# SudYar/MLVectorDB

Hardware: AMD Instinct MI355X
Metric: queries/sec, exact cosine kNN k=10 over a row-sharded Nx768 fp32 corpus (10M rows per GPU) (higher is better)
Workload: dtype i8 (MFMA bounds) + f64 (exact rescoring of the f32 rows)

## Files before the change

### mlvectordb_amd/csrc/kernels_filter.hip

```cpp
#include <cstdlib>
#include <type_traits>

#include "bound_common.h"
#include "internal.h"
#include "query_norm.h"
#include "scan_common.h"

namespace mlvdb {

typedef __bf16 bf16x8 __attribute__((ext_vector_type(8)));
typedef float f32x4 __attribute__((ext_vector_type(4)));
typedef int i32x4 __attribute__((ext_vector_type(4)));
typedef float f32x8 __attribute__((ext_vector_type(8)));
typedef unsigned int u32x4 __attribute__((ext_vector_type(4)));

__device__ __forceinline__ __amdgpu_buffer_rsrc_t make_rsrc(const void* base, uint32_t bytes) {
    return __builtin_amdgcn_make_buffer_rsrc(const_cast<void*>(base), 0, bytes, 0x00020000);
}
__device__ __forceinline__ float4 buf_load_f4(__amdgpu_buffer_rsrc_t r, uint32_t voff, uint32_t soff) {
    return __builtin_bit_cast(float4, __builtin_amdgcn_raw_buffer_load_b128(r, voff, soff, 0));
}
__device__ __forceinline__ float4 buf_load_f4_nt(__amdgpu_buffer_rsrc_t r, uint32_t voff, uint32_t soff) {
    return __builtin_bit_cast(float4, __builtin_amdgcn_raw_buffer_load_b128(r, voff, soff, 2));
}
// ... 1564 lines not shown
        const float v = x * invf;
        const __bf16 b = (__bf16)v;
        int kc = c >> 6, ks, g, j;
        if (a.Xb) {
            ks = (c >> 5) & 1; g = (c >> 3) & 3; j = c & 7;
        } else {
            const int t = (c >> 4) & 3;
            ks = t >> 1; g = (c >> 2) & 3; j = (t & 1) * 4 + (c & 3);
        }
        if (want_bf16) img[((((int64_t)kc * 16 + n16) * 2 + ks) * 64 + (c16 + 16 * g)) * 8 + j] = b;
        if (c < dim) {
            const double e = (double)x * inv - (double)(float)(__bf16)(x * invf);
            e2 = __builtin_fma(e, e, e2);
        }
        amax = __builtin_fmaxf(amax, __builtin_fabsf(v));
    }
    for (int off = 32; off > 0; off >>= 1) {
        e2 += __shfl_xor(e2, off);
        amax = __builtin_fmaxf(amax, __shfl_xor(amax, off));
    }
    __syncthreads();
    if (lane == 0) {
        dred[wave] = e2;
        fred[wave] = amax;
    }
    __syncthreads();
    if (threadIdx.x == 0) {
        float e = (float)(__builtin_sqrt((dred[0] + dred[1]) + (dred[2] + dred[3])) * 1.000001);
        e = float_bump(e);
        if (real) qerr[q] = e;
        const double nrm = live ? (a.space == kSpaceCosine ? 0.0 : qaux[q]) : 0.0;
        a.qscale[q] = a.space == kSpaceL2 ? (float)(2.0 * nrm) : 1.0f;
        const double e1q = (real ? (double)e : 0.0) + 1.00390625 * (double)*a.row_err + (double)ld * 2.384185791015625e-07;
        const float ke = (float)(e1q * 1.000001) + (a.space == kSpaceCosine ? 2.0f : 1.0f) * kSlack;
        a.ke[q] = float_bump(ke);
        a.thr[q] = real ? -3.0e38f : 3.4e38f;
        a.cnt[q] = 0;
        a.overflow[q] = s_flag ? 1u : 0u;
    }
    if (!want_i8) return;
    amax = __builtin_fmaxf(__builtin_fmaxf(fred[0], fred[1]), __builtin_fmaxf(fred[2], fred[3]));
    if (a.l2c) {
        if (threadIdx.x == 0) a.rmaxq[q] = live ? float_above((double)amax * (qaux[q] + 1e-30) * 1.000001) : 0.f;
        return;
    }
    const float sq = amax > 0.f ? amax / 127.0f : 1.0f;
    const float isq = 1.0f / sq;
    int8_t* img8 = reinterpret_cast<int8_t*>(a.qimg8);
    double err2 = 0.0;
    for (int c = threadIdx.x; c < a.ld8; c += 256) {
        const float v = live && c < ld ? dst[c] * invf : 0.f;
        float t = __builtin_rintf(v * isq);
        t = __builtin_fminf(127.f, __builtin_fmaxf(-127.f, t));
        const double e = (double)v - (double)sq * (double)t;
        err2 += e * e;
        const int kc = c >> 7, ks = (c >> 6) & 1, g = (c >> 4) & 3, j = c & 15;
        img8[((((int64_t)kc * 16 + n16) * 2 + ks) * 64 + (c16 + 16 * g)) * 16 + j] = (int8_t)t;
    }
    for (int off = 32; off > 0; off >>= 1) err2 += __shfl_xor(err2, off);
    __syncthreads();
    if (lane == 0) dred[wave] = err2;
    __syncthreads();
    if (threadIdx.x == 0) {
        const double eq8 = __builtin_sqrt(dred[0] + dred[1] + dred[2] + dred[3]) * 1.000001 + 1e-12;
        a.sq8[q] = sq;
        a.ke8[q] = real ? float_above(eq8) : 0.f;
        if (real && a.nq > 1) {
            atomicMin(a.sqmin, __float_as_uint(sq));
            atomicMax(a.sqmin + 1, __float_as_uint(float_above(eq8)));
        }
        if (real && a.nq == 1) {
            prep8_fin_query(a, 0, sq, float_above(eq8));
        }
    }
    if (want_i8 && a.nq == 1 && q > 0 && threadIdx.x == 0) prep8_fin_query(a, q, 1.0f, 0.0f);
}

__global__ __launch_bounds__(256) void filter_prep8_l2c_kernel(const FilterArgs a) {
    __shared__ double dred[4];
    const int q = blockIdx.x;
    const int ld = a.ld;
    const int lane = threadIdx.x & 63, wave = threadIdx.x >> 6;
    const bool real = q < a.nq;
    __shared__ __attribute__((aligned(16))) unsigned long long s_key[kFilterQueries];
    __shared__ float s_q[2];
    const float rmax_t = (int)threadIdx.x < a.nq ? a.rmaxq[threadIdx.x] : -1.f;
    {
        const unsigned long long key = rank_key_256(rmax_t, (int)threadIdx.x);
        s_key[threadIdx.x] = key;
        __syncthreads();
        if (rmax_t >= 0.f && rank_among_256(s_key, key) == (a.nq - 1) / 2) s_q[0] = rmax_t;
    }
    __syncthreads();
    {
        const float cap = s_q[0] > 0.f ? 4.0f * s_q[0] : 3.0e38f;
        float v = rmax_t;
        v = (v >= 0.f && v <= cap) ? v : 0.f;
        for (int off = 32; off > 0; off >>= 1) v = __builtin_fmaxf(v, __shfl_xor(v, off));
        if ((threadIdx.x & 63) == 0) dred[threadIdx.x >> 6] = (double)v;
    }
    __syncthreads();
    float qmax = (float)__builtin_fmax(__builtin_fmax(dred[0], dred[1]), __builtin_fmax(dred[2], dred[3]));
    __syncthreads();
    if (qmax > 0.f && qmax < 1.0e30f) {
        float g = exp2f(ceilf(log2f(qmax) * 4.0f) * 0.25f);
        if (g < qmax) g *= 1.18920712f;
        if (g >= qmax && g <= qmax * 1.5f) qmax = g;
    }
    const float SQ = qmax > 0.f ? float_above((double)qmax * (2.0 / 127.0) * 1.000001) : 1.0f;
    const bool live = real && a.overflow[q] == 0u;
    const double nrm = live ? a.qaux[q] : 0.0;
    const float invf = (float)(1.0 / (nrm + 1e-30));
    const float sq = nrm > 0.0 ? (float)((double)SQ / (2.0 * nrm)) : 1.0f;
    const float isq = 1.0f / sq;
    int8_t* img8 = reinterpret_cast<int8_t*>(a.qimg8);
    const int n16 = q >> 4, c16 = q & 15;
    double err2 = 0.0;
    for (int c = threadIdx.x; c < a.ld8; c += 256) {
        const float v = live && c < ld ? a.Qpad[(int64_t)q * ld + c] * invf : 0.f;
        float t = __builtin_rintf(v * isq);
        t = __builtin_fminf(127.f, __builtin_fmaxf(-127.f, t));
        const double e = (double)v - (double)sq * (double)t;
        err2 += e * e;
        const int kc = c >> 7, ks = (c >> 6) & 1, g = (c >> 4) & 3, j = c & 15;
        img8[((((int64_t)kc * 16 + n16) * 2 + ks) * 64 + (c16 + 16 * g)) * 16 + j] = (int8_t)t;
    }
    for (int off = 32; off > 0; off >>= 1) err2 += __shfl_xor(err2, off);
    if (lane == 0) dred[wave] = err2;
    __syncthreads();
    if (threadIdx.x == 0) {
        const double eq8 = __builtin_sqrt(dred[0] + dred[1] + dred[2] + dred[3]) * 1.000001 + 1e-12;
        a.sq8[q] = sq;
        a.ke8[q] = real ? float_above(eq8) : 0.f;
        prep8_fin_query(a, q, 1.0f, 0.0f);
    }
}

hipError_t launch_filter_prep_fused(const FilterArgs& a, const float* queries, int32_t dim, float* Qpad, double* qaux, float* qerr,
                                    hipStream_t s) {
    const int want_i8 = a.X8 != nullptr;
    if (!want_i8 && !filter_supported(a.ld)) return hipErrorInvalidValue;
    filter_prep_fused_kernel<<<kFilterQueries, 256, 0, s>>>(a, queries, dim, Qpad, qaux, qerr, want_i8);
    if (want_i8 && a.l2c) filter_prep8_l2c_kernel<<<kFilterQueries, 256, 0, s>>>(a);
    else if (want_i8 && a.nq > 1) filter_prep8_fin_kernel<<<1, kFilterQueries, 0, s>>>(a, 1);
    return hipGetLastError();
}

hipError_t launch_filter_prep8(const FilterArgs& a, hipStream_t s) {
    filter_prep8_kernel<<<kFilterQueries, 256, 0, s>>>(a);
    filter_prep8_fin_kernel<<<1, kFilterQueries, 0, s>>>(a, 1);
    return hipGetLastError();
}

__device__ __forceinline__ uint32_t radix_select_atleast256(const uint32_t* keys, uint32_t cnt, uint32_t want, uint32_t cap,
                                                            uint32_t kmin, uint32_t kmax, uint32_t* hist, uint32_t* s_sel,
                                                            uint32_t* ties, uint32_t* total) {
    const int lane = threadIdx.x & 63, wave = threadIdx.x >> 6;
    const uint32_t want0 = want;
    const uint32_t diff = kmin ^ kmax;
    uint32_t prefix = kmax, mask = 0xffffffffu;
    if (diff != 0) {
        const int hb = 31 - __builtin_clz(diff);
        mask = hb == 31 ? 0u : ~((2u << hb) - 1u);
        prefix = kmax & mask;
        int shift = hb >= 7 ? hb - 7 : 0, width = hb - shift + 1;
        for (;;) {
            __syncthreads();
            hist[threadIdx.x] = 0;
            __syncthreads();
            const uint32_t dmask = (1u << width) - 1u;
            for (uint32_t idx = threadIdx.x; idx < cnt; idx += 256) {
                const uint32_t key = keys[idx];
                if (key != 0 && (key & mask) == prefix) atomicAdd(&hist[(key >> shift) & dmask], 1u);
            }
            __syncthreads();
            if (wave == 0) {
                const uint32_t h0 = hist[4 * lane], h1 = hist[4 * lane + 1], h2 = hist[4 * lane + 2], h3 = hist[4 * lane + 3];
                uint32_t above = h0 + h1 + h2 + h3;
                uint32_t run = above;
                for (int off = 1; off < 64; off <<= 1) {
                    const uint32_t v = __shfl_down(run, off);
                    if (lane + off < 64) run += v;
                }
                above = run - above;
                const uint32_t c3 = above + h3, c2 = c3 + h2, c1 = c2 + h1, c0 = c1 + h0;
                if (above < want && c0 >= want) {
                    if (c3 >= want) { s_sel[0] = 4 * lane + 3; s_sel[1] = above; s_sel[2] = h3; }
                    else if (c2 >= want) { s_sel[0] = 4 * lane + 2; s_sel[1] = c3; s_sel[2] = h2; }
                    else if (c1 >= want) { s_sel[0] = 4 * lane + 1; s_sel[1] = c2; s_sel[2] = h1; }
                    else { s_sel[0] = 4 * lane; s_sel[1] = c1; s_sel[2] = h0; }
                }
            }
            __syncthreads();
            prefix |= s_sel[0] << shift;
            mask |= dmask << shift;
            want -= s_sel[1];
            if (want0 - want + s_sel[2] <= cap) {
                *ties = 0xffffffffu;
                *total = want0 - want + s_sel[2];
                return prefix;
            }
            if (shift == 0) break;
            const int next = shift >= 8 ? shift - 8 : 0;
            width = shift - next;
            shift = next;
        }
        *ties = want;
        *total = want0;
        return prefix;
    }
    *ties = want;
    *total = want0;
    return prefix;
}

template <int kPer>
__global__ __launch_bounds__(256) void filter_prefix_thr_kernel(const FilterArgs a, const double* __restrict__ d64, const int32_t m,
                                                                const int32_t k) {
    __shared__ __attribute__((aligned(16))) uint32_t tmax[256];
    __shared__ uint32_t sel[256];
    __shared__ uint32_t s_n[4];
    const int q = blockIdx.x;
    const double aux = a.qaux[q];
    if (a.l2c && a.overflow[q]) return;
    if (a.space == kSpaceIp && !(aux > 0.0)) return;
    uint32_t key[kPer], best = 0;
    double dk[kPer];
#pragma unroll
    for (int j = 0; j < kPer; ++j) {
        const int i = j * 256 + threadIdx.x;
        dk[j] = i < m ? d64[(int64_t)q * m + i] : __builtin_inf();
    }
#pragma unroll
    for (int j = 0; j < kPer; ++j) {
        key[j] = 0;
        if (dk[j] < 1.0e300) {
            double s;
            if (a.space == kSpaceCosine) s = 1.0 - dk[j];
            else if (a.space == kSpaceIp) s = (1.0 - dk[j]) / aux;
            else s = aux * aux - dk[j];
            const double mag = a.space == kSpaceL2 ? aux * aux + __builtin_fabs(dk[j]) : __builtin_fabs(s) + 1.0;
            key[j] = float_order_key(float_below(s - 1e-9 * mag));
            if (key[j] == 0) key[j] = 1;
            best = max(best, key[j]);
        }
    }
    tmax[threadIdx.x] = best;
    if (threadIdx.x < 4) s_n[threadIdx.x] = 0;
    __syncthreads();
    if (k <= 256) {
        uint32_t rank = 0;
        const uint4* t4 = reinterpret_cast<const uint4*>(tmax);
        const uint32_t me = threadIdx.x;
#pragma unroll 8
        for (uint32_t j = 0; j < 64; ++j) {
            const uint4 o = t4[j];
            rank += (o.x > best || (o.x == best && 4 * j < me)) ? 1u : 0u;
            rank += (o.y > best || (o.y == best && 4 * j + 1 < me)) ? 1u : 0u;
            rank += (o.z > best || (o.z == best && 4 * j + 2 < me)) ? 1u : 0u;
            rank += (o.w > best || (o.w == best && 4 * j + 3 < me)) ? 1u : 0u;
        }
        if (rank == (uint32_t)k - 1u) s_n[1] = best;
    }
    __syncthreads();
    const uint32_t L = s_n[1];
    if (L == 0) return;
#pragma unroll
    for (int j = 0; j < kPer; ++j)
        if (key[j] >= L) {
            const uint32_t pos = atomicAdd(&s_n[0], 1u);
            if (pos < 256u) sel[pos] = key[j];
        }
    __syncthreads();
    const uint32_t n = s_n[0];
    uint32_t tkey = L;
    if (n <= 256u) {
        if (threadIdx.x < n) {
            const uint32_t mine = sel[threadIdx.x];
            uint32_t rank = 0;
            for (uint32_t j = 0; j < n; ++j) {
                const uint32_t o = sel[j];
                rank += (o > mine || (o == mine && j < threadIdx.x)) ? 1u : 0u;
            }
            if (rank == (uint32_t)k - 1u) s_n[2] = mine;
        }
        __syncthreads();
        tkey = s_n[2];
    }
    if (threadIdx.x == 0) a.thr[q] = float_from_order_key(tkey);
}

hipError_t launch_filter_prefix_thr(const FilterArgs& a, const double* d64, int32_t m, int32_t k, hipStream_t s) {
    if (m < 1 || m > 3 * kSeedRows || k < 1 || k > 256) return hipErrorInvalidValue;
    if (m <= kSeedRows) filter_prefix_thr_kernel<kSeedRows / 256><<<a.nq, 256, 0, s>>>(a, d64, m, k);
    else filter_prefix_thr_kernel<3 * kSeedRows / 256><<<a.nq, 256, 0, s>>>(a, d64, m, k);
    return hipGetLastError();
}

struct FinishOut {
    int32_t q0;
    int64_t* labels;
    float* dist;
    int32_t* counts;
    double* d64;
    unsigned long long* rescored;
    int32_t* qsel;
    int32_t* nflag;
};

template <int SPACE, bool FINISH = false>
__global__ __launch_bounds__(256) void filter_refine_thr_kernel(const FilterArgs a, const int32_t k, const int32_t forced_cnt,
                                                                const bool fuse, const int32_t picks, const FinishOut fo) {
    extern __shared__ __attribute__((aligned(16))) char smem[];
    double* qs = reinterpret_cast<double*>(smem);
    double* sc = qs + a.ld;
    double* smin = sc + 64;
    int32_t* pick = reinterpret_cast<int32_t*>(smin + 1);
    uint32_t* hist = reinterpret_cast<uint32_t*>(pick + 64);
    uint32_t* s_scan = hist + 256;
    uint32_t* keys = s_scan + 24;
    CandEntry* stage = reinterpret_cast<CandEntry*>(keys + kCandCap);
    const int q = blockIdx.x;
    if (FINISH && blockIdx.x == 0 && fo.qsel) {
        uint32_t* s_flagged = s_scan + 18;
        const int t = threadIdx.x;
        const bool flagged = t < a.nq && (a.overflow[t] != 0 || a.cnt[t] > (uint32_t)kCandCap);
        const unsigned long long bal = __ballot(flagged);
        if ((t & 63) == 0) s_flagged[t >> 6] = __popcll(bal);
        __syncthreads();
        int base = 0;
        for (int w = 0; w < (t >> 6); ++w) base += (int)s_flagged[w];
        if (flagged) fo.qsel[base + __popcll(bal & ((1ull << (t & 63)) - 1ull))] = t;
        if (t == 0) {
            const int n = (int)(s_flagged[0] + s_flagged[1] + s_flagged[2] + s_flagged[3]);
            *fo.nflag = n;
            if (fo.rescored) fo.rescored[1] += (unsigned long long)n;
        }
    }
    if (q >= a.nq || a.overflow[q]) return;
    const uint32_t cnt = forced_cnt >= 0 ? (uint32_t)forced_cnt : a.cnt[q];
    if (cnt > (uint32_t)kCandCap) {
        if (fuse && threadIdx.x == 0) a.overflow[q] = 1u;
        return;
    }
    bool ok = cnt >= (uint32_t)k && k <= 64;
    if (!ok && !fuse) return;
    const int ld = a.ld;
    const int lane = threadIdx.x & 63, wave = threadIdx.x >> 6;
    CandEntry* list = a.cand + (int64_t)q * kCandCap;
    for (int c = threadIdx.x; c < ld; c += 256) qs[c] = (double)a.Qpad[(int64_t)q * ld + c];
    uint32_t n_valid = 0, kmin = 0xffffffffu, kmax = 0;
    for (uint32_t base = 0; base < cnt; base += 256 * 8) {
        CandEntry e[8];
#pragma unroll
        for (int j = 0; j < 8; ++j) {
            const uint32_t idx = base + j * 256 + threadIdx.x;
            e[j] = list[idx < cnt ? idx : cnt - 1];
        }
#pragma unroll
        for (int j = 0; j < 8; ++j) {
            const uint32_t idx = base + j * 256 + threadIdx.x;
            if (idx >= cnt) continue;
            if (fuse) stage[idx] = e[j];
            uint32_t key = 0;
            if (e[j].u == e[j].u) {
                key = float_order_key(e[j].u);
                if (key == 0) key = 1;
                ++n_valid;
                kmin = min(kmin, key);
                kmax = max(kmax, key);
            }
            keys[idx] = key;
        }
    }
    for (int off = 32; off > 0; off >>= 1) {
        n_valid += __shfl_xor(n_valid, off);
        kmin = min(kmin, (uint32_t)__shfl_xor(kmin, off));
        kmax = max(kmax, (uint32_t)__shfl_xor(kmax, off));
    }
    if (lane == 0) {
        s_scan[wave] = n_valid;
        s_scan[4 + wave] = kmin;
        s_scan[8 + wave] = kmax;
    }
    __syncthreads();
    n_valid = s_scan[0] + s_scan[1] + s_scan[2] + s_scan[3];
    kmin = min(min(s_scan[4], s_scan[5]), min(s_scan[6], s_scan[7]));
    kmax = max(max(s_scan[8], s_scan[9]), max(s_scan[10], s_scan[11]));
    if (n_valid < (uint32_t)k) ok = false;
    uint32_t m = 0;
    if (ok) {
        const uint32_t want = min((uint32_t)max(picks, k), 64u), cap = max(want, 32u);
        uint32_t tkey = 1, ties = 0xffffffffu;
        m = n_valid;
        if (n_valid > cap) tkey = radix_select_atleast256(keys, cnt, want, cap, kmin, kmax, hist, s_scan + 12, &ties, &m);
        if (threadIdx.x == 0) s_scan[16] = 0;
        __syncthreads();
        const bool split = ties != 0xffffffffu;
        for (uint32_t idx = threadIdx.x; idx < cnt; idx += 256) {
            const uint32_t key = keys[idx];
            if (key != 0 && (split ? key > tkey : key >= tkey)) {
                const uint32_t pos = atomicAdd(&s_scan[16], 1u);
                if (pos < 64u) pick[pos] = fuse ? stage[idx].row : list[idx].row;
            }
        }
        if (split && wave == 0) {
            uint32_t taken = 0;
            const uint32_t above = m - ties;
            for (uint32_t base = 0; base < cnt && taken < ties; base += 64) {
                const uint32_t idx = base + lane;
                const bool hit = idx < cnt && keys[idx] == tkey;
                const unsigned long long bal = __ballot(hit);
                const uint32_t pos = taken + (uint32_t)__popcll(bal & ((1ull << lane) - 1ull));
                if (hit && pos < ties && above + pos < 64u) pick[above + pos] = fuse ? stage[idx].row : list[idx].row;
                taken += (uint32_t)__popcll(bal);
            }
        }
    }
    __syncthreads();
    if (ok) m = min(m, 64u);
    const int rslot = threadIdx.x >> 3, l8 = threadIdx.x & 7;
    const double qinv = a.qaux[q];
    const int ngroups = ld >> 4;
    constexpr int G = 6;
    for (uint32_t p0 = 0; p0 < m; p0 += 32) {
        const uint32_t pidx = p0 + rslot;
        const bool have = pidx < m;
        const int32_t row = have ? pick[pidx] : pick[0];
        const float* rb = a.X + (int64_t)(row >> 4) * (kPanelRows * ld) + (row & 15) * 16;
        double acc = 0.0, nx = 0.0;
        for (int c0 = l8; c0 < ngroups; c0 += 8 * G) {
            float4 v[G][4];
#pragma unroll
            for (int j = 0; j < G; ++j) {
                const int cg = c0 + 8 * j < ngroups ? c0 + 8 * j : c0;
                const float4* src = reinterpret_cast<const float4*>(rb + (int64_t)cg * kGroupFloats);
#pragma unroll
                for (int i = 0; i < 4; ++i) v[j][i] = src[i];
            }
#pragma unroll
            for (int j = 0; j < G; ++j) {
                if (c0 + 8 * j >= ngroups) continue;
                const double* qp = qs + (c0 + 8 * j) * 16;
#pragma unroll
                for (int i = 0; i < 4; ++i) {
                    const double x[4] = {(double)v[j][i].x, (double)v[j][i].y, (double)v[j][i].z, (double)v[j][i].w};
#pragma unroll
                    for (int t = 0; t < 4; ++t) {
                        if (SPACE == kSpaceL2) {
                            const double e = qp[4 * i + t] - x[t];
                            acc = __builtin_fma(e, e, acc);
                        } else {
                            acc = __builtin_fma(qp[4 * i + t], x[t], acc);
                        }
                        if (SPACE == kSpaceCosine) nx = __builtin_fma(x[t], x[t], nx);
                    }
                }
            }
        }
        for (int off = 1; off < 8; off <<= 1) {
            acc += __shfl_xor(acc, off);
            if (SPACE == kSpaceCosine) nx += __shfl_xor(nx, off);
        }
        const double dk = finish_distance<SPACE>(acc, nx, qinv);
        double s;
        if (SPACE == kSpaceCosine) s = 1.0 - dk;
        else if (SPACE == kSpaceIp) s = (1.0 - dk) / qinv;
        else s = qinv * qinv - dk;
        if (have && l8 == 0) sc[pidx] = s == s ? s : -__builtin_inf();
    }
    if (threadIdx.x == 0) *smin = -__builtin_inf();
    __syncthreads();
    if (ok && threadIdx.x < m) {
        const double si = sc[threadIdx.x];
        uint32_t rank = 0;
        for (uint32_t j = 0; j < m; ++j) {
            const double sj = sc[j];
            rank += (sj > si || (sj == si && j < threadIdx.x)) ? 1u : 0u;
        }
        if (rank == (uint32_t)k - 1u) *smin = si;
    }
    __syncthreads();
    float thr = a.thr[q];
    if (ok) {
        const double sm = *smin;
        if (sm > -1.0e300 && sm < 1.0e300) {
            const double mag = SPACE == kSpaceL2 ? qinv * qinv + __builtin_fabs(sm) : __builtin_fabs(sm) + 1.0;
            const float t = float_below(sm - 1e-9 * mag);
            if (t > thr) thr = t;
        }
    }
    if (!fuse) {
        if (threadIdx.x == 0) a.thr[q] = thr;
        return;
    }
    const uint32_t per = ((cnt + 255u) / 256u) * 64u;
    const uint32_t wb = min(cnt, (uint32_t)wave * per), we = min(cnt, wb + per);
    uint32_t keep = 0;
    for (uint32_t base = wb; base < we; base += 64) {
        const uint32_t idx = base + lane;
        keep += (uint32_t)__popcll(__ballot(idx < we && stage[idx].u >= thr));
    }
    if (lane == 0) s_scan[wave] = keep;
    __syncthreads();
    uint32_t pos = 0;
    for (int w = 0; w < wave; ++w) pos += s_scan[w];
    const uint32_t new_cnt = s_scan[0] + s_scan[1] + s_scan[2] + s_scan[3];
    uint32_t* surv = keys;
    if (FINISH || new_cnt != cnt) {
        for (uint32_t base = wb; base < we; base += 64) {
            const uint32_t idx = base + lane;
            const bool kept = idx < we && stage[idx].u >= thr;
            const unsigned long long bal = __ballot(kept);
            const uint32_t at = pos + (uint32_t)__popcll(bal & ((1ull << lane) - 1ull));
            if (kept) {
                if (FINISH) surv[at] = (uint32_t)stage[idx].row;
                else list[at] = stage[idx];
            }
            pos += (uint32_t)__popcll(bal);
        }
    }
    if (threadIdx.x == 0) {
        a.thr[q] = thr;
        a.cnt[q] = new_cnt;
    }
    if (!FINISH) return;
    __syncthreads();
    constexpr int kFinWaves = 4;
    double* ed = reinterpret_cast<double*>(stage);
    int32_t* el = reinterpret_cast<int32_t*>(ed + kRescoreRankMax);
    RangeHit* rs = a.rs + (int64_t)q * kCandCap;
    const bool in_lds = new_cnt <= (uint32_t)kRescoreRankMax;
    {
        const int g = lane >> 4, r = lane & 15;
        for (uint32_t base = (uint32_t)wave * 16; base < new_cnt; base += kFinWaves * 16) {
            const uint32_t idx = base + r;
            const bool have = idx < new_cnt;
            const int32_t row = (int32_t)surv[have ? idx : base];
            const float* rbase[1] = {a.X + (int64_t)(row >> 4) * (kPanelRows * ld) + (row & 15) * 16 + g * 4};
            double acc[1][1], nx[1];
            accumulate_rows<SPACE, 1, 1, kRescorePF>(rbase, qs, ld, g, acc, nx);
            const double dist = finish_distance<SPACE>(acc[0][0], nx[0], qinv);
            if (have && lane < 16) {
                const float nrm = a.rn[row];
                const bool live = nrm == nrm;
                if (in_lds) {
                    ed[idx] = live ? dist : __builtin_inf();
                    el[idx] = live ? row : kNoLabel;
                } else {
                    RangeHit hit;
                    hit.d = live ? dist : __builtin_inf();
                    hit.l = live ? row : kNoLabel;
                    hit.pad = 0;
                    rs[idx] = hit;
                }
            }
        }
    }
    if (threadIdx.x == 0) s_scan[17] = 0;
    __syncthreads();
    const int64_t o = (int64_t)(fo.q0 + q) * k;
    if (in_lds) {
        int mine = 0;
        for (uint32_t i = wave; i < new_cnt; i += kFinWaves) {
            const double di = ed[i];
            const int32_t li = el[i];
            if (li == kNoLabel) continue;
            ++mine;
            int rank = 0;
            for (uint32_t j0 = 0; j0 < new_cnt && rank < k; j0 += 128) {
                const uint32_t j = j0 + lane, j2 = j + 64;
                const bool l0 = j < new_cnt && entry_less(ed[j], el[j], di, li);
                const bool l1 = j2 < new_cnt && entry_less(ed[j2], el[j2], di, li);
                rank += __popcll(__ballot(l0)) + __popcll(__ballot(l1));
            }
            if (lane == 0 && rank < k) {
                fo.labels[o + rank] = (int64_t)li;
                fo.dist[o + rank] = (float)di;
                if (fo.d64) fo.d64[o + rank] = di;
            }
        }
        if (lane == 0 && mine) atomicAdd(&s_scan[17], (uint32_t)mine);
        __syncthreads();
        const int n_out = min((int)s_scan[17], k);
        for (int i = n_out + threadIdx.x; i < k; i += 256) {
            fo.labels[o + i] = -1;
            fo.dist[o + i] = __builtin_inff();
            if (fo.d64) fo.d64[o + i] = __builtin_inf();
        }
        if (threadIdx.x == 0) {
            fo.counts[fo.q0 + q] = n_out;
            if (fo.rescored) atomicAdd(fo.rescored, (unsigned long long)new_cnt);
        }
        return;
    }
    double* sd = reinterpret_cast<double*>(stage);
    int32_t* sl = reinterpret_cast<int32_t*>(sd + kFinWaves * 64);
    WaveTopK top;
    top.init();
    for (uint32_t b = 0; b < new_cnt; b += kFinWaves * 64) {
        const uint32_t i = b + wave * 64 + lane;
        RangeHit hh;
        hh.d = __builtin_inf();
        hh.l = kNoLabel;
        if (i < new_cnt) hh = rs[i];
        top.offer(hh.l != kNoLabel, hh.d, hh.l, k, lane);
    }
    sd[wave * 64 + lane] = top.d;
    sl[wave * 64 + lane] = top.l;
    __syncthreads();
    if (wave != 0) return;
    WaveTopK f;
    f.init();
#pragma unroll
    for (int w2 = 0; w2 < kFinWaves; ++w2)
        f.offer(lane < k && sl[w2 * 64 + lane] != kNoLabel, sd[w2 * 64 + lane], sl[w2 * 64 + lane], k, lane);
    const bool valid = lane < k && f.l != kNoLabel;
    if (lane < k) {
        fo.labels[o + lane] = valid ? (int64_t)f.l : -1;
        fo.dist[o + lane] = valid ? (float)f.d : __builtin_inff();
        if (fo.d64) fo.d64[o + lane] = valid ? f.d : __builtin_inf();
    }
    const int n_valid_out = __popcll(__ballot(valid));
    if (lane == 0) {
        fo.counts[fo.q0 + q] = n_valid_out;
        if (fo.rescored) atomicAdd(fo.rescored, (unsigned long long)new_cnt);
    }
}

bool filter_refine_can_fuse(const FilterArgs& a) { return a.ld <= 2048; }

hipError_t launch_filter_refine_thr(const FilterArgs& a, int32_t k, int32_t forced_cnt, bool fuse, hipStream_t s) {
    const size_t lds = (size_t)a.ld * sizeof(double) + 65 * sizeof(double) + 64 * 4 + 256 * 4 + 24 * 4 + (size_t)kCandCap * 4 +
                       (fuse ? (size_t)kCandCap * sizeof(CandEntry) : 0);
    auto kern = a.space == kSpaceL2 ? filter_refine_thr_kernel<kSpaceL2>
                : a.space == kSpaceCosine ? filter_refine_thr_kernel<kSpaceCosine> : filter_refine_thr_kernel<kSpaceIp>;
    static std::atomic<uint64_t> configured[3];
    if (hipError_t e = ensure_dynamic_lds(configured[a.space], reinterpret_cast<const void*>(kern), 160 * 1024); e != hipSuccess)
        return e;
    const int pv = a.tn ? a.tn->refine_picks : 0;
    int picks = pv > 0 ? pv : k + k / 2;
    if (pv <= 0 && picks < 16) picks = 16;
    picks = picks < k ? k : (picks > 64 ? 64 : picks);
    kern<<<a.nq, 256, lds, s>>>(a, k, forced_cnt, fuse, picks, FinishOut{});
    return hipGetLastError();
}

hipError_t launch_filter_finish_small(const FilterArgs& a, int32_t k, int32_t q0, int64_t* out_labels, float* out_dist,
                                      int32_t* out_counts, double* out_d64, unsigned long long* rescored, int32_t* qsel,
                                      int32_t* nflag, hipStream_t s) {
    if (!filter_refine_can_fuse(a) || k < 1 || k > 64) return hipErrorInvalidValue;
    const size_t lds = (size_t)a.ld * sizeof(double) + 65 * sizeof(double) + 64 * 4 + 256 * 4 + 24 * 4 + (size_t)kCandCap * 4 +
                       (size_t)kCandCap * sizeof(CandEntry);
    auto kern = a.space == kSpaceL2 ? filter_refine_thr_kernel<kSpaceL2, true>
                : a.space == kSpaceCosine ? filter_refine_thr_kernel<kSpaceCosine, true> : filter_refine_thr_kernel<kSpaceIp, true>;
    static std::atomic<uint64_t> configured[3];
    if (hipError_t e = ensure_dynamic_lds(configured[a.space], reinterpret_cast<const void*>(kern), 160 * 1024); e != hipSuccess)
        return e;
    const int pv = a.tn ? a.tn->refine_picks : 0;
    int picks = pv > 0 ? pv : k + k / 2;
    if (pv <= 0 && picks < 16) picks = 16;
    picks = picks < k ? k : (picks > 64 ? 64 : picks);
    FinishOut fo{q0, out_labels, out_dist, out_counts, out_d64, rescored, qsel, nflag};
    kern<<<a.nq, 256, lds, s>>>(a, k, -1, true, picks, fo);
    return hipGetLastError();
}

template <int SPACE, bool XB, bool DENSE = false>
static hipError_t launch_scan_one(const FilterArgs& a, int64_t row_begin, int64_t row_end, hipStream_t s) {
    constexpr int NW = 4, MT = 2;
    constexpr int tile_rows = NW * 16 * MT;
    const int64_t tile_begin = row_begin / tile_rows;
    const int64_t tile_end = (row_end + tile_rows - 1) / tile_rows;
    if (tile_end <= tile_begin) return hipSuccess;
    const size_t lds = 2 * kChunkVec * sizeof(uint4) + 3 * kFilterQueries * sizeof(float) +
                       (size_t)NW * 4 * MT * 64 * sizeof(float);
    const int64_t ntiles = tile_end - tile_begin;
    const int max_grid = 256 * 2;
    const int grid = (int)(ntiles < max_grid ? ntiles : max_grid);
    auto kern = filter_scan_kernel<SPACE, XB, DENSE>;
    static std::atomic<uint64_t> configured{0};
    if (hipError_t e = ensure_dynamic_lds(configured, reinterpret_cast<const void*>(kern), (int)lds); e != hipSuccess)
        return e;
    kern<<<grid, NW * 64, lds, s>>>(a, tile_begin, tile_end);
    return hipGetLastError();
}

constexpr int kNarrowMaxQueries = 64;
constexpr size_t kNarrowLdsMax = 152 * 1024;
static int narrow_nqt(int nq) { return nq <= 16 ? 1 : (nq <= 32 ? 2 : 4); }
static size_t narrow_lds(int32_t ld, int nqt, int nw, bool i8 = false) {
    return (size_t)(ld / (i8 ? 64 : 32)) * nqt * 1024 + 3 * kFilterQueries * sizeof(float) + (size_t)nw * 4 * 2 * 64 * sizeof(float);
}
bool filter_narrow_ok(const FilterArgs& a) {
    if (!a.Xb || a.X8 || a.nq > kNarrowMaxQueries) return false;
    if (a.tn->scan_narrow == 0) return false;
    return narrow_lds(a.ld, narrow_nqt(a.nq), 8) <= kNarrowLdsMax;
}
template <int SPACE, int NQT, bool DENSE, int R, int NW, bool I8 = false>
static hipError_t launch_scan_narrow_n(const FilterArgs& a, int64_t row_begin, int64_t row_end, hipStream_t s, int qgroups = 1) {
    constexpr int tile_rows = NW * 32;
    const int64_t tile_begin = row_begin / tile_rows;
    const int64_t tile_end = (row_end + tile_rows - 1) / tile_rows;
    if (tile_end <= tile_begin) return hipSuccess;
    const size_t lds = narrow_lds(I8 ? a.ld8 : a.ld, NQT, NW, I8);
    const int64_t ntiles = tile_end - tile_begin;
    const int per_cu = (int)std::min<size_t>(32 / NW, (160 * 1024) / lds);
    const int max_grid = 256 * per_cu;
    const int64_t rounds = (ntiles + max_grid - 1) / max_grid;
    const int grid = (int)((ntiles + rounds - 1) / rounds);
    auto kern = filter_scan_narrow_kernel<SPACE, NQT, DENSE, R, NW, I8>;
    static std::atomic<uint64_t> configured{0};
    if (hipError_t e = ensure_dynamic_lds(configured, reinterpret_cast<const void*>(kern), (int)kNarrowLdsMax); e != hipSuccess)
        return e;
    kern<<<dim3((unsigned)grid, (unsigned)qgroups), NW * 64, lds, s>>>(a, tile_begin, tile_end);
    return hipGetLastError();
}
template <int SPACE, int NQT, bool DENSE>
static hipError_t launch_scan_narrow_q(const FilterArgs& a, int64_t row_begin, int64_t row_end, hipStream_t s) {
    const bool r4 = (a.ld / 32) % 4 == 0;
    if constexpr (DENSE) {
        return r4 ? launch_scan_narrow_n<SPACE, NQT, true, 4, 4>(a, row_begin, row_end, s)
                  : launch_scan_narrow_n<SPACE, NQT, true, 2, 4>(a, row_begin, row_end, s);
    } else {
        return r4 ? launch_scan_narrow_n<SPACE, NQT, false, 4, 8>(a, row_begin, row_end, s)
                  : launch_scan_narrow_n<SPACE, NQT, false, 2, 8>(a, row_begin, row_end, s);
    }
}
template <int SPACE, bool DENSE>
static hipError_t launch_scan_narrow(const FilterArgs& a, int64_t row_begin, int64_t row_end, hipStream_t s) {
    switch (narrow_nqt(a.nq)) {
        case 1: return launch_scan_narrow_q<SPACE, 1, DENSE>(a, row_begin, row_end, s);
        case 2: return launch_scan_narrow_q<SPACE, 2, DENSE>(a, row_begin, row_end, s);
        default: return launch_scan_narrow_q<SPACE, 4, DENSE>(a, row_begin, row_end, s);
    }
}

template <int SPACE, int R, bool I8, int NQT = 16, int QB = kAsmQBufs>
static hipError_t launch_scan_asm(const FilterArgs& a, int64_t row_begin, int64_t row_end, hipStream_t s) {
    constexpr int NW = kAsmWaves, tile_rows = NW * 32;
    const int64_t tile_begin = row_begin / tile_rows;
    const int64_t tile_end = (row_end + tile_rows - 1) / tile_rows;
    if (tile_end <= tile_begin) return hipSuccess;
    constexpr int stage_cap = QB == 4 ? kAsmQ4StageCap : kAsmStageCap;
    constexpr size_t lds = QB * kChunkVec * sizeof(uint4) + 3 * kFilterQueries * sizeof(float) + (size_t)NW * 12 * stage_cap;
    static_assert(lds <= 160 * 1024, "one workgroup per CU");
    const int64_t ntiles = tile_end - tile_begin;
    const int max_grid = 256;
    const int grid = (int)(ntiles < max_grid ? ntiles : max_grid);
    auto kern = filter_scan_asm_kernel<SPACE, R, I8, NQT, QB>;
    static std::atomic<uint64_t> configured{0};
    static std::atomic<int> lds_base_ok{0};
    if (lds_base_ok.load(std::memory_order_acquire) == 0) {
        hipFuncAttributes attr{};
        if (hipError_t e = hipFuncGetAttributes(&attr, reinterpret_cast<const void*>(kern)); e != hipSuccess) return e;
        lds_base_ok.store(attr.sharedSizeBytes == 0 ? 1 : -1, std::memory_order_release);
    }
    if (lds_base_ok.load(std::memory_order_acquire) < 0) return hipErrorInvalidConfiguration;
    if (hipError_t e = ensure_dynamic_lds(configured, reinterpret_cast<const void*>(kern), (int)lds); e != hipSuccess)
        return e;
    kern<<<grid, NW * 64, lds, s>>>(a, tile_begin, tile_end, 0);
    return hipGetLastError();
}

template <int SPACE>
static hipError_t launch_scan_space(const FilterArgs& a, int64_t row_begin, int64_t row_end, hipStream_t s) {
    if (filter_narrow_ok(a)) return launch_scan_narrow<SPACE, false>(a, row_begin, row_end, s);
    if (a.X8 && a.ld8 > 0) {
        const int nqt = a.tn->scan_nqt > 0 ? a.tn->scan_nqt : (a.nq <= 64 ? 4 : (a.nq <= 128 ? 8 : 16));
        if (nqt <= 4 && a.nq <= 64) return launch_scan_asm<SPACE, 4, true, 4>(a, row_begin, row_end, s);
        if (nqt <= 8 && a.nq <= 128) return launch_scan_asm<SPACE, 4, true, 8>(a, row_begin, row_end, s);
        if (a.scan_q4 && a.nq > 128 && a.ld8 == kAsmQ4Chunks * 2 * kFilterChunkK)
            return launch_scan_asm<SPACE, 4, true, 16, 4>(a, row_begin, row_end, s);
        return launch_scan_asm<SPACE, 4, true, 16>(a, row_begin, row_end, s);
    }
    if (a.Xb) {
        if ((a.ld / kFilterChunkK) % 2 == 0) return launch_scan_asm<SPACE, 4, false>(a, row_begin, row_end, s);
        return launch_scan_asm<SPACE, 2, false>(a, row_begin, row_end, s);
    }
    return launch_scan_one<SPACE, false>(a, row_begin, row_end, s);
}

static hipError_t launch_update(const FilterArgs& a, int32_t k, int32_t forced_cnt, hipStream_t s);

hipError_t launch_filter_dense_scan(const FilterArgs& a, int64_t rows, hipStream_t s) {
    const bool xb = a.Xb != nullptr;
    if (filter_narrow_ok(a)) {
// ... 129 lines not shown
```

Before: 143,100.

## Keep refine-kernel candidates and radix keys in registers instead of LDS

The threshold-refine kernel now holds candidate entries and their order keys in per-thread register arrays. The array size is picked from three compile-time variants based on the candidate count. The radix select, tie-breaking and compaction work from these registers through a shared ballot-based list-order helper, which replaces the LDS keys/stage arrays and the global reloads. The first candidate slots are loaded speculatively before the query copy to overlap latency, and the rank loop is batched. This cuts LDS traffic and the dynamic LDS size, which could allow more resident blocks. The cost is higher register pressure, three template instantiations, and possible spills at the largest slot count.

```diff
diff --git a/mlvectordb_amd/csrc/kernels_filter.hip b/mlvectordb_amd/csrc/kernels_filter.hip
--- a/mlvectordb_amd/csrc/kernels_filter.hip
+++ b/mlvectordb_amd/csrc/kernels_filter.hip
@@ -1740,9 +1740,13 @@
     return hipGetLastError();
 }
 
-__device__ __forceinline__ uint32_t radix_select_atleast256(const uint32_t* keys, uint32_t cnt, uint32_t want, uint32_t cap,
-                                                            uint32_t kmin, uint32_t kmax, uint32_t* hist, uint32_t* s_sel,
-                                                            uint32_t* ties, uint32_t* total) {
+constexpr int kRefineSlots = kCandCap / 256;
+constexpr int kRefineEarly = 8;
+
+template <int NS>
+__device__ __forceinline__ uint32_t radix_select_atleast256(const uint32_t (&kreg)[NS], uint32_t cnt, uint32_t want,
+                                                            uint32_t cap, uint32_t kmin, uint32_t kmax, uint32_t* hist,
+                                                            uint32_t* s_sel, uint32_t* ties, uint32_t* total) {
     const int lane = threadIdx.x & 63, wave = threadIdx.x >> 6;
     const uint32_t want0 = want;
     const uint32_t diff = kmin ^ kmax;
@@ -1753,12 +1757,11 @@
         prefix = kmax & mask;
         int shift = hb >= 7 ? hb - 7 : 0, width = hb - shift + 1;
         for (;;) {
-            __syncthreads();
-            hist[threadIdx.x] = 0;
-            __syncthreads();
             const uint32_t dmask = (1u << width) - 1u;
-            for (uint32_t idx = threadIdx.x; idx < cnt; idx += 256) {
-                const uint32_t key = keys[idx];
+#pragma unroll
+            for (int j = 0; j < NS; ++j) {
+                if ((uint32_t)j * 256u >= cnt) continue;
+                const uint32_t key = kreg[j];
                 if (key != 0 && (key & mask) == prefix) atomicAdd(&hist[(key >> shift) & dmask], 1u);
             }
             __syncthreads();
@@ -1792,6 +1795,8 @@
             const int next = shift >= 8 ? shift - 8 : 0;
             width = shift - next;
             shift = next;
+            hist[threadIdx.x] = 0;
+            __syncthreads();
         }
         *ties = want;
         *total = want0;
@@ -1800,6 +1805,37 @@
     *ties = want;
     *total = want0;
     return prefix;
+}
+
+template <int NS, class Flag, class Emit>
+__device__ __forceinline__ uint32_t refine_in_list_order(uint32_t cnt, uint32_t* cnts, Flag flag, Emit emit) {
+    const int lane = threadIdx.x & 63, wave = threadIdx.x >> 6;
+#pragma unroll
+    for (int j = 0; j < NS; ++j) {
+        if ((uint32_t)j * 256u >= cnt) continue;
+        const unsigned long long bal = __ballot(flag(j));
+        if (lane == 0) cnts[4 * j + wave] = (uint32_t)__popcll(bal);
+    }
+    __syncthreads();
+    uint32_t total = 0;
+#pragma unroll
+    for (int j = 0; j < NS; ++j) {
+        if ((uint32_t)j * 256u >= cnt) continue;
+        total += cnts[4 * j] + cnts[4 * j + 1] + cnts[4 * j + 2] + cnts[4 * j + 3];
+    }
+    uint32_t base = 0;
+#pragma unroll
+    for (int j = 0; j < NS; ++j) {
+        if ((uint32_t)j * 256u >= cnt) continue;
+        const uint32_t c0 = cnts[4 * j], c1 = cnts[4 * j + 1], c2 = cnts[4 * j + 2], c3 = cnts[4 * j + 3];
+        const bool f = flag(j);
+        const unsigned long long bal = __ballot(f);
+        const uint32_t at = base + (wave > 0 ? c0 : 0u) + (wave > 1 ? c1 : 0u) + (wave > 2 ? c2 : 0u) +
+                            (uint32_t)__popcll(bal & ((1ull << lane) - 1ull));
+        if (f) emit(j, at, total);
+        base += c0 + c1 + c2 + c3;
+    }
+    return total;
 }
 
 template <int kPer>
@@ -1906,8 +1942,8 @@
     int32_t* pick = reinterpret_cast<int32_t*>(smin + 1);
     uint32_t* hist = reinterpret_cast<uint32_t*>(pick + 64);
     uint32_t* s_scan = hist + 256;
-    uint32_t* keys = s_scan + 24;
-    CandEntry* stage = reinterpret_cast<CandEntry*>(keys + kCandCap);
+    uint32_t* surv = s_scan + 24;
+    CandEntry* stage = reinterpret_cast<CandEntry*>(surv + kCandCap);
     const int q = blockIdx.x;
     if (FINISH && blockIdx.x == 0 && fo.qsel) {
         uint32_t* s_flagged = s_scan + 18;
@@ -1925,40 +1961,83 @@
             if (fo.rescored) fo.rescored[1] += (unsigned long long)n;
         }
     }
-    if (q >= a.nq || a.overflow[q]) return;
-    const uint32_t cnt = forced_cnt >= 0 ? (uint32_t)forced_cnt : a.cnt[q];
+    if (q >= a.nq) return;
+    const int ld = a.ld;
+    const int lane = threadIdx.x & 63, wave = threadIdx.x >> 6;
+    CandEntry* list = a.cand + (int64_t)q * kCandCap;
+    const uint32_t flagged_q = a.overflow[q];
+    const uint32_t cnt_q = a.cnt[q];
+    const float thr0 = a.thr[q];
+    const double qinv = a.qaux[q];
+    CandEntry e0[2 * kRefineEarly];
+#pragma unroll
+    for (int j = 0; j < kRefineEarly; ++j) e0[j] = list[j * 256 + threadIdx.x];
+    const uint32_t cnt_told = forced_cnt >= 0 ? min((uint32_t)forced_cnt, (uint32_t)(2 * kRefineEarly * 256)) : 0u;
+#pragma unroll
+    for (int j = kRefineEarly; j < 2 * kRefineEarly; ++j) {
+        if ((uint32_t)j * 256u >= cnt_told) continue;
+        const uint32_t idx = (uint32_t)j * 256u + threadIdx.x;
+        e0[j] = list[idx < cnt_told ? idx : cnt_told - 1];
+    }
+    for (int c0 = 0; c0 < ld; c0 += 4 * 256) {
+        float v[4];
+#pragma unroll
+        for (int j = 0; j < 4; ++j) {
+            const int c = c0 + j * 256 + threadIdx.x;
+            v[j] = a.Qpad[(int64_t)q * ld + (c < ld ? c : ld - 1)];
+        }
+#pragma unroll
+        for (int j = 0; j < 4; ++j) {
+            const int c = c0 + j * 256 + threadIdx.x;
+            if (c < ld) qs[c] = (double)v[j];
+        }
+    }
+    if (flagged_q) return;
+    const uint32_t cnt = forced_cnt >= 0 ? (uint32_t)forced_cnt : cnt_q;
     if (cnt > (uint32_t)kCandCap) {
         if (fuse && threadIdx.x == 0) a.overflow[q] = 1u;
         return;
     }
-    bool ok = cnt >= (uint32_t)k && k <= 64;
-    if (!ok && !fuse) return;
-    const int ld = a.ld;
-    const int lane = threadIdx.x & 63, wave = threadIdx.x >> 6;
-    CandEntry* list = a.cand + (int64_t)q * kCandCap;
-    for (int c = threadIdx.x; c < ld; c += 256) qs[c] = (double)a.Qpad[(int64_t)q * ld + c];
+    const bool ok0 = cnt >= (uint32_t)k && k <= 64;
+    if (!ok0 && !fuse) return;
+    auto body = [&](auto slots) {
+    constexpr int NS = decltype(slots)::value;
+    bool ok = ok0;
+    CandEntry e[NS];
+#pragma unroll
+    for (int j = 0; j < NS; ++j) {
+        if (j < kRefineEarly || (j < 2 * kRefineEarly && (uint32_t)j * 256u < cnt_told)) {
+            e[j] = e0[j];
+            continue;
+        }
+        if ((uint32_t)j * 256u >= cnt) continue;
+        const uint32_t idx = (uint32_t)j * 256u + threadIdx.x;
+        e[j] = list[idx < cnt ? idx : cnt - 1];
+    }
+    hist[threadIdx.x] = 0;
+    if (threadIdx.x == 0) {
+        s_scan[16] = 0;
+        *smin = -__builtin_inf();
+    }
+    uint32_t kreg[NS];
     uint32_t n_valid = 0, kmin = 0xffffffffu, kmax = 0;
-    for (uint32_t base = 0; base < cnt; base += 256 * 8) {
-        CandEntry e[8];
-#pragma unroll
-        for (int j = 0; j < 8; ++j) {
-            const uint32_t idx = base + j * 256 + threadIdx.x;
-            e[j] = list[idx < cnt ? idx : cnt - 1];
-        }
-#pragma unroll
-        for (int j = 0; j < 8; ++j) {
-            const uint32_t idx = base + j * 256 + threadIdx.x;
-            if (idx >= cnt) continue;
-            if (fuse) stage[idx] = e[j];
-            uint32_t key = 0;
-            if (e[j].u == e[j].u) {
-                key = float_order_key(e[j].u);
-                if (key == 0) key = 1;
-                ++n_valid;
-                kmin = min(kmin, key);
-                kmax = max(kmax, key);
-            }
-            keys[idx] = key;
+    const float qnan = __builtin_nanf("");
+#pragma unroll
+    for (int j = 0; j < NS; ++j) {
+        kreg[j] = 0;
+        if ((uint32_t)j * 256u >= cnt) {
+            e[j].u = qnan;
+            e[j].row = 0;
+            continue;
+        }
+        if ((uint32_t)j * 256u + threadIdx.x >= cnt) e[j].u = qnan;
+        if (e[j].u == e[j].u) {
+            uint32_t key = float_order_key(e[j].u);
+            if (key == 0) key = 1;
+            ++n_valid;
+            kmin = min(kmin, key);
+            kmax = max(kmax, key);
+            kreg[j] = key;
         }
     }
     for (int off = 32; off > 0; off >>= 1) {
@@ -1981,34 +2060,29 @@
         const uint32_t want = min((uint32_t)max(picks, k), 64u), cap = max(want, 32u);
         uint32_t tkey = 1, ties = 0xffffffffu;
         m = n_valid;
-        if (n_valid > cap) tkey = radix_select_atleast256(keys, cnt, want, cap, kmin, kmax, hist, s_scan + 12, &ties, &m);
-        if (threadIdx.x == 0) s_scan[16] = 0;
-        __syncthreads();
+        if (n_valid > cap) tkey = radix_select_atleast256<NS>(kreg, cnt, want, cap, kmin, kmax, hist, s_scan + 12, &ties, &m);
         const bool split = ties != 0xffffffffu;
-        for (uint32_t idx = threadIdx.x; idx < cnt; idx += 256) {
-            const uint32_t key = keys[idx];
+#pragma unroll
+        for (int j = 0; j < NS; ++j) {
+            if ((uint32_t)j * 256u >= cnt) continue;
+            const uint32_t key = kreg[j];
             if (key != 0 && (split ? key > tkey : key >= tkey)) {
                 const uint32_t pos = atomicAdd(&s_scan[16], 1u);
-                if (pos < 64u) pick[pos] = fuse ? stage[idx].row : list[idx].row;
-            }
-        }
-        if (split && wave == 0) {
-            uint32_t taken = 0;
+                if (pos < 64u) pick[pos] = e[j].row;
+            }
+        }
+        if (split) {
             const uint32_t above = m - ties;
-            for (uint32_t base = 0; base < cnt && taken < ties; base += 64) {
-                const uint32_t idx = base + lane;
-                const bool hit = idx < cnt && keys[idx] == tkey;
-                const unsigned long long bal = __ballot(hit);
-                const uint32_t pos = taken + (uint32_t)__popcll(bal & ((1ull << lane) - 1ull));
-                if (hit && pos < ties && above + pos < 64u) pick[above + pos] = fuse ? stage[idx].row : list[idx].row;
-                taken += (uint32_t)__popcll(bal);
-            }
+            refine_in_list_order<NS>(
+                cnt, hist, [&](int j) { return kreg[j] == tkey; },
+                [&](int j, uint32_t at, uint32_t) {
+                    if (at < ties && above + at < 64u) pick[above + at] = e[j].row;
+                });
         }
     }
     __syncthreads();
     if (ok) m = min(m, 64u);
     const int rslot = threadIdx.x >> 3, l8 = threadIdx.x & 7;
-    const double qinv = a.qaux[q];
     const int ngroups = ld >> 4;
     constexpr int G = 6;
     for (uint32_t p0 = 0; p0 < m; p0 += 32) {
@@ -2036,8 +2110,8 @@
 #pragma unroll
                     for (int t = 0; t < 4; ++t) {
                         if (SPACE == kSpaceL2) {
-                            const double e = qp[4 * i + t] - x[t];
-                            acc = __builtin_fma(e, e, acc);
+                            const double df = qp[4 * i + t] - x[t];
+                            acc = __builtin_fma(df, df, acc);
                         } else {
                             acc = __builtin_fma(qp[4 * i + t], x[t], acc);
                         }
@@ -2057,19 +2131,24 @@
         else s = qinv * qinv - dk;
         if (have && l8 == 0) sc[pidx] = s == s ? s : -__builtin_inf();
     }
-    if (threadIdx.x == 0) *smin = -__builtin_inf();
     __syncthreads();
     if (ok && threadIdx.x < m) {
         const double si = sc[threadIdx.x];
         uint32_t rank = 0;
-        for (uint32_t j = 0; j < m; ++j) {
-            const double sj = sc[j];
-            rank += (sj > si || (sj == si && j < threadIdx.x)) ? 1u : 0u;
+        for (uint32_t j0 = 0; j0 < m; j0 += 8) {
+            double sj[8];
+#pragma unroll
+            for (uint32_t t = 0; t < 8; ++t) sj[t] = sc[j0 + t];
+#pragma unroll
+            for (uint32_t t = 0; t < 8; ++t) {
+                const uint32_t j = j0 + t;
+                rank += (j < m && (sj[t] > si || (sj[t] == si && j < threadIdx.x))) ? 1u : 0u;
+            }
         }
         if (rank == (uint32_t)k - 1u) *smin = si;
     }
     __syncthreads();
-    float thr = a.thr[q];
+    float thr = thr0;
     if (ok) {
         const double sm = *smin;
         if (sm > -1.0e300 && sm < 1.0e300) {
@@ -2082,32 +2161,12 @@
         if (threadIdx.x == 0) a.thr[q] = thr;
         return;
     }
-    const uint32_t per = ((cnt + 255u) / 256u) * 64u;
-    const uint32_t wb = min(cnt, (uint32_t)wave * per), we = min(cnt, wb + per);
-    uint32_t keep = 0;
-    for (uint32_t base = wb; base < we; base += 64) {
-        const uint32_t idx = base + lane;
-        keep += (uint32_t)__popcll(__ballot(idx < we && stage[idx].u >= thr));
-    }
-    if (lane == 0) s_scan[wave] = keep;
-    __syncthreads();
-    uint32_t pos = 0;
-    for (int w = 0; w < wave; ++w) pos += s_scan[w];
-    const uint32_t new_cnt = s_scan[0] + s_scan[1] + s_scan[2] + s_scan[3];
-    uint32_t* surv = keys;
-    if (FINISH || new_cnt != cnt) {
-        for (uint32_t base = wb; base < we; base += 64) {
-            const uint32_t idx = base + lane;
-            const bool kept = idx < we && stage[idx].u >= thr;
-            const unsigned long long bal = __ballot(kept);
-            const uint32_t at = pos + (uint32_t)__popcll(bal & ((1ull << lane) - 1ull));
-            if (kept) {
-                if (FINISH) surv[at] = (uint32_t)stage[idx].row;
-                else list[at] = stage[idx];
-            }
-            pos += (uint32_t)__popcll(bal);
-        }
-    }
+    const uint32_t new_cnt = refine_in_list_order<NS>(
+        cnt, hist, [&](int j) { return e[j].u >= thr; },
+        [&](int j, uint32_t at, uint32_t total) {
+            if (FINISH) surv[at] = (uint32_t)e[j].row;
+            else if (total != cnt) list[at] = e[j];
+        });
     if (threadIdx.x == 0) {
         a.thr[q] = thr;
         a.cnt[q] = new_cnt;
@@ -2214,13 +2273,16 @@
         fo.counts[fo.q0 + q] = n_valid_out;
         if (fo.rescored) atomicAdd(fo.rescored, (unsigned long long)new_cnt);
     }
+    };
+    if (cnt <= 8u * 256u) body(std::integral_constant<int, 8>{});
+    else if (cnt <= 16u * 256u) body(std::integral_constant<int, 16>{});
+    else body(std::integral_constant<int, kRefineSlots>{});
 }
 
 bool filter_refine_can_fuse(const FilterArgs& a) { return a.ld <= 2048; }
 
 hipError_t launch_filter_refine_thr(const FilterArgs& a, int32_t k, int32_t forced_cnt, bool fuse, hipStream_t s) {
-    const size_t lds = (size_t)a.ld * sizeof(double) + 65 * sizeof(double) + 64 * 4 + 256 * 4 + 24 * 4 + (size_t)kCandCap * 4 +
-                       (fuse ? (size_t)kCandCap * sizeof(CandEntry) : 0);
+    const size_t lds = (size_t)a.ld * sizeof(double) + 65 * sizeof(double) + 64 * 4 + 256 * 4 + 24 * 4;
     auto kern = a.space == kSpaceL2 ? filter_refine_thr_kernel<kSpaceL2>
                 : a.space == kSpaceCosine ? filter_refine_thr_kernel<kSpaceCosine> : filter_refine_thr_kernel<kSpaceIp>;
     static std::atomic<uint64_t> configured[3];
```

New measurement: 143,500, median of 6. Within noise of the previous version (+0.3%).
